# ooowedyn/InkLayer

Hardware: AMD Instinct MI355X
Metric: sketches/sec end-to-end (GroundingDINO+SAM) at 1024x1024 (higher is better)
Workload: dtype f16 (MFMA, f32 accumulate; f32 residual/norm/softmax; split-f16 = fp32-grade operands for patch-embed, neck, mask decoder)

## Files before the change

inklayer_amd/csrc/attention.hip:

```cpp
#include <stdlib.h>
#include "common.h"
#include "../../include/inklayer_hip.h"

int ink_win4_attn_launch(const InkAttn& p, int n_cus, hipStream_t s);
int ink_glob4_attn_launch(const InkAttn& p, hipStream_t s);

namespace {

typedef __attribute__((address_space(3))) s16x4* lds_s16x4_ptr;

__device__ __forceinline__ f16x4 tr_read(const char* p) {
  s16x4 v = __builtin_amdgcn_ds_read_tr16_b64_v4i16((lds_s16x4_ptr)(p));
  return __builtin_bit_cast(f16x4, v);
}

__device__ __forceinline__ f16x8 cvt8(const f32x16& s, int base) {
  f16x8 r;
#pragma unroll
  for (int j = 0; j < 8; ++j) r[j] = (f16)s[base + j];
  return r;
}

__device__ __forceinline__ float max3(float a, float b, float c) {
  float d;
  asm("v_max3_f32 %0, %1, %2, %3" : "=v"(d) : "v"(a), "v"(b), "v"(c));
  return d;
}

template <int HD, int MODE, int NW, bool ALLKV = false>
__global__ __launch_bounds__(NW * 64) void flash_attn_kernel(InkAttn p) {
  constexpr int NQKB = HD / 16;
  constexpr int NQK = NQKB + (MODE == 2 ? 2 : 0);
  constexpr int NB = (HD + 31) / 32;
  constexpr int DVP = NB * 32;
  constexpr bool LSUM_MFMA = DVP >= HD + 8;
  constexpr int CH = HD / 8;
  constexpr int KROW = ((NQK * 2) | 1) * 16;
  constexpr int VROW = DVP * 2;
  constexpr int NT = NW * 64;
  constexpr int KIT = (64 * CH + NT - 1) / NT;
  constexpr float NEG = -1e30f;
  constexpr int TILEB = 64 * KROW + 64 * VROW;
  constexpr int MAXT = ALLKV ? 4 : 2;
  extern __shared__ __attribute__((aligned(16))) char smem[];
  char* sK = smem;
  char* sV = smem + 64 * KROW;
  char* sR = smem + MAXT * TILEB;

  const int tid = threadIdx.x, lane = tid & 63, wave = tid >> 6;
  const int lq = lane & 31, hh = lane >> 5;
  const int nqb = (p.n_q + NW * 32 - 1) / (NW * 32);
  const int total = p.n_batch * p.n_heads * nqb;
  int blk = ALLKV ? (int)((int64_t)blockIdx.x * total / gridDim.x)
                  : (MODE == 1 ? xcd_remap((int)blockIdx.x, (int)gridDim.x) : (int)blockIdx.x);
  const int blk_end = ALLKV ? (int)((int64_t)(blockIdx.x + 1) * total / gridDim.x) : blk + 1;

  struct QState { bool ok; int64_t row; };
  constexpr int KALL = ALLKV ? (MAXT * 64 * CH + NT - 1) / NT : 1;
  int wrow_q = 0, wrow_k[KALL], wrow_b = -1;
  auto load_wrows = [&](int b_) {
    if (MODE == 2 && ALLKV && p.tok_rows && b_ != wrow_b) {
      const int qi = wave * 32 + lq;
      wrow_q = p.tok_rows[(int64_t)b_ * p.n_q + (qi < p.n_q ? qi : p.n_q - 1)];
#pragma unroll
      for (int it = 0; it < KALL; ++it) {
        const int key = (tid + it * NT) / CH;
        wrow_k[it] = key < p.n_k ? p.tok_rows[(int64_t)b_ * p.n_k + key] : -1;
      }
      wrow_b = b_;
    }
  };
  auto load_q = [&](int blk_, f16x8 (&dst)[NQK]) -> QState {
    const int bh_ = blk_ / nqb, qb_ = blk_ % nqb;
    const int b_ = bh_ / p.n_heads, h_ = bh_ % p.n_heads;
    const int qi = qb_ * NW * 32 + wave * 32 + lq;
    bool ok = qi < p.n_q;
    const int qc = ok ? qi : p.n_q - 1;
    const int64_t qrow0 = p.q_batch_rows ? (int64_t)p.q_batch_rows[b_] : (int64_t)b_ * p.n_q;
    int64_t row = qrow0 + qc;
    if constexpr (MODE == 2 && ALLKV) {
      if (p.tok_rows) {
        ok = ok && wrow_q >= 0;
        row = wrow_q >= 0 ? wrow_q : 0;
      }
    }
    const f16* Qrow = (const f16*)p.Q + row * p.ldq + h_ * HD;
#pragma unroll
    for (int s = 0; s < NQKB; ++s) dst[s] = *(const f16x8*)(Qrow + 16 * s + 8 * hh);
    if constexpr (MODE == 2) {
      const f16* R = (const f16*)p.rel_aug + ((int64_t)bh_ * p.n_q + qc) * 32;
      dst[NQKB] = *(const f16x8*)(R + 8 * hh);
      dst[NQKB + 1] = *(const f16x8*)(R + 16 + 8 * hh);
    }
    return QState{ok, row};
  };
  f16x8 ka[KALL], va[KALL];
  (void)ka; (void)va;
  auto load_kv_all = [&](int blk_) {
    const int bh_ = blk_ / nqb;
    const int b_ = bh_ / p.n_heads, h_ = bh_ % p.n_heads;
    const int64_t kvb_ = p.kv_batch_rows ? (int64_t)p.kv_batch_rows[b_] : (int64_t)b_ * p.n_k;
#pragma unroll
    for (int it = 0; it < KALL; ++it) {
      const int ci = tid + it * NT;
      const int key = ci / CH, cc = ci % CH;
      ka[it] = (f16x8){0, 0, 0, 0, 0, 0, 0, 0};
      va[it] = (f16x8){0, 0, 0, 0, 0, 0, 0, 0};
      if (ci < MAXT * 64 * CH && key < p.n_k) {
        int64_t r = kvb_ + key;
        if (MODE == 2 && p.tok_rows) r = wrow_k[it];
        if (r >= 0) {
          ka[it] = *(const f16x8*)((const f16*)p.K + r * p.ldk + h_ * HD + cc * 8);
          va[it] = *(const f16x8*)((const f16*)p.V + r * p.ldv + h_ * HD + cc * 8);
        } else {
          ka[it] = *(const f16x8*)((const f16*)p.pad_k + h_ * HD + cc * 8);
          va[it] = *(const f16x8*)((const f16*)p.pad_v + h_ * HD + cc * 8);
        }
      }
    }
  };
  load_wrows((blk / nqb) / p.n_heads);
  f16x8 qf[NQK];
  QState qs = load_q(blk, qf);
  if constexpr (ALLKV) load_kv_all(blk);
  if constexpr (DVP > HD) {
    constexpr int PCH = (DVP - HD) / 8;
    for (int i = tid; i < MAXT * 64 * PCH; i += NT) {
      const int row = (i / PCH) % 64, pc = i % PCH, tl = i / (64 * PCH);
      f16x8 z = {0, 0, 0, 0, 0, 0, 0, 0};
      if (LSUM_MFMA && pc == 0) { z[0] = (f16)1; z[4] = (f16)1; }
      *(f16x8*)(sV + tl * TILEB + row * VROW + (CH + pc) * 16) = z;
    }
  }
  int koff_g[KIT], voff_g[KIT], loff_k[KIT], loff_v[KIT];
#pragma unroll
  for (int it = 0; it < KIT; ++it) {
    const int ci = tid + it * NT;
    const int row = (ci / CH) & 63, cc = ci % CH;
    koff_g[it] = (row * (int)p.ldk + cc * 8) * 2;
    voff_g[it] = (row * (int)p.ldv + cc * 8) * 2;
    loff_k[it] = row * KROW + cc * 16;
    loff_v[it] = row * VROW + cc * 16;
  }
  if constexpr (MODE == 2 && ALLKV) {
    for (int i = tid; i < MAXT * 256; i += NT) {
      const int key = i >> 2, c4 = i & 3;
      const int kh = key / p.grid_w, kw = key - kh * p.grid_w + p.grid_w;
      f16x8 e;
#pragma unroll
      for (int j = 0; j < 8; ++j) {
        const int col = c4 * 8 + j;
        e[j] = (key < p.n_k && (col == kh || col == kw)) ? (f16)1 : (f16)0;
      }
      *(f16x8*)(sK + (key >> 6) * TILEB + (key & 63) * KROW + (CH + c4) * 16) = e;
    }
  }
  const float c = p.scale * 1.44269504088896340736f;
  const int ntiles = (p.n_k + 63) / 64;
  const bool half_tail = ALLKV && (p.n_k - (ntiles - 1) * 64) <= 32;
  const int koff0 = lq * KROW + hh * 16;
  const int koff1 = (32 + lq) * KROW + hh * 16;
  const int voff = (4 * hh + ((lane & 15) >> 2)) * VROW + (16 * ((lane >> 4) & 1) + 4 * (lane & 3)) * 2;
  constexpr int LI = HD / 32, LR = (((HD % 32) / 8) * 4);

  for (; blk < blk_end; ++blk) {
  const int bh = blk / nqb, qb = blk % nqb;
  const int b = bh / p.n_heads, h = bh % p.n_heads;
  const int q_idx = qb * NW * 32 + wave * 32 + lq;
  const int q_c = q_idx < p.n_q ? q_idx : p.n_q - 1;
  const bool q_ok = qs.ok;
  const int64_t q_row = qs.row;
  const int64_t kvb = p.kv_batch_rows ? (int64_t)p.kv_batch_rows[b] : (int64_t)b * p.n_k;
  const char* Kb = (const char*)((const f16*)p.K + kvb * p.ldk + h * HD);
  const char* Vb = (const char*)((const f16*)p.V + kvb * p.ldv + h * HD);
  float bias3[2][16];
  const float* RH = nullptr;
  if constexpr (MODE == 3) {
    const float* bp = p.dense_bias + ((int64_t)h * p.n_q + q_c) * 64;
    const float* mp = p.dense_mask ? p.dense_mask + ((int64_t)(b % p.n_mask) * p.n_q + q_c) * 64 : nullptr;
#pragma unroll
    for (int sub = 0; sub < 2; ++sub)
#pragma unroll
      for (int g = 0; g < 4; ++g) {
        f32x4 v = *(const f32x4*)(bp + sub * 32 + 8 * g + 4 * hh);
        if (mp) v += *(const f32x4*)(mp + sub * 32 + 8 * g + 4 * hh);
#pragma unroll
        for (int r = 0; r < 4; ++r) bias3[sub][4 * g + r] = v[r];
      }
  }
  f32x16 rw0, rw1;
  if constexpr (MODE == 1) {
    const float* RW = p.rel_w + ((int64_t)bh * p.n_q + q_c) * 64;
    RH = p.rel_h + ((int64_t)bh * p.n_q + q_c) * 64;
#pragma unroll
    for (int g = 0; g < 4; ++g) {
      const f32x4 a = *(const f32x4*)(RW + 8 * g + 4 * hh), c2 = *(const f32x4*)(RW + 32 + 8 * g + 4 * hh);
#pragma unroll
      for (int r = 0; r < 4; ++r) { rw0[4 * g + r] = a[r]; rw1[4 * g + r] = c2[r]; }
    }
  }

  f16x8 kreg[KIT], vreg[KIT];
  auto load_tile = [&](int t) {
    const char* kt = Kb + (int64_t)t * 64 * p.ldk * 2;
    const char* vt = Vb + (int64_t)t * 64 * p.ldv * 2;
    const bool full = (t + 1) * 64 <= p.n_k;
#pragma unroll
    for (int it = 0; it < KIT; ++it) {
      const int ci = tid + it * NT;
      const bool ok = ci < 64 * CH && (full || t * 64 + ci / CH < p.n_k);
      if (ok) {
        kreg[it] = *(const f16x8*)(kt + koff_g[it]);
        vreg[it] = *(const f16x8*)(vt + voff_g[it]);
      } else {
        kreg[it] = (f16x8){0, 0, 0, 0, 0, 0, 0, 0};
        vreg[it] = (f16x8){0, 0, 0, 0, 0, 0, 0, 0};
      }
    }
  };
  auto store_tile = [&](int t) {
#pragma unroll
    for (int it = 0; it < KIT; ++it) {
      if (tid + it * NT < 64 * CH) {
        *(f16x8*)(sK + (t & 1) * TILEB + loff_k[it]) = kreg[it];
        *(f16x8*)(sV + (t & 1) * TILEB + loff_v[it]) = vreg[it];
      }
    }
    if constexpr (MODE == 2 && !ALLKV) {
      for (int i = tid; i < 256; i += NT) {
        const int row = i >> 2, c4 = i & 3;
        const int key = t * 64 + row;
        const int kh = key / p.grid_w, kw = key - kh * p.grid_w + p.grid_w;
        f16x8 e;
#pragma unroll
        for (int j = 0; j < 8; ++j) {
          const int col = c4 * 8 + j;
          e[j] = (key < p.n_k && (col == kh || col == kw)) ? (f16)1 : (f16)0;
        }
        *(f16x8*)(sK + (t & 1) * TILEB + row * KROW + (CH + c4) * 16) = e;
      }
    }
  };

  f32x16 o[NB];
#pragma unroll
  for (int i = 0; i < NB; ++i)
#pragma unroll
    for (int r = 0; r < 16; ++r) o[i][r] = 0.f;
  float m_run = NEG, l_run = 0.f;

  float rh_next = 0.f;
  if constexpr (MODE == 1) rh_next = RH[0];
  if constexpr (ALLKV) {
    __syncthreads();
#pragma unroll
    for (int it = 0; it < KALL; ++it) {
      const int ci = tid + it * NT;
      const int key = ci / CH, cc = ci % CH;
      if (ci < MAXT * 64 * CH) {
        *(f16x8*)(sK + (key >> 6) * TILEB + (key & 63) * KROW + cc * 16) = ka[it];
        *(f16x8*)(sV + (key >> 6) * TILEB + (key & 63) * VROW + cc * 16) = va[it];
      }
    }
    __syncthreads();
    if (blk + 1 < blk_end) {
      load_wrows(((blk + 1) / nqb) / p.n_heads);
      load_kv_all(blk + 1);
    }
  } else {
    load_tile(0);
    store_tile(0);
    if (ntiles > 1) load_tile(1);
    __syncthreads();
  }
  const int nt_wave = (ALLKV && !__any(q_ok)) ? 0 : ntiles;
  for (int t = 0; t < nt_wave; ++t) {
    const char* tK = sK + (ALLKV ? t : (t & 1)) * TILEB;
    const char* tV = sV + (ALLKV ? t : (t & 1)) * TILEB;
    const float rh = rh_next;
    if constexpr (MODE == 1) {
      if (t + 1 < ntiles) rh_next = RH[t + 1];
    }

    f32x16 s0, s1;
    constexpr bool KPRE = !ALLKV;
    f16x8 kfa[KPRE ? NQK : 1], kfb[KPRE ? NQK : 1];
    if constexpr (KPRE) {
#pragma unroll
      for (int s = 0; s < NQK; ++s) {
        kfa[s] = *(const f16x8*)(tK + koff0 + s * 32);
        kfb[s] = *(const f16x8*)(tK + koff1 + s * 32);
      }
      __builtin_amdgcn_sched_barrier(0);
    }
    if constexpr (MODE == 1) {
      s0 = __builtin_amdgcn_mfma_f32_32x32x16_f16(kfa[0], qf[0], rw0, 0, 0, 0);
      s1 = __builtin_amdgcn_mfma_f32_32x32x16_f16(kfb[0], qf[0], rw1, 0, 0, 0);
    } else if constexpr (MODE == 3) {
#pragma unroll
      for (int r = 0; r < 16; ++r) {
        s0[r] = bias3[0][r];
        s1[r] = bias3[1][r];
      }
    } else {
#pragma unroll
      for (int r = 0; r < 16; ++r) s0[r] = s1[r] = 0.f;
    }
    const bool half = half_tail && t == ntiles - 1;
    if (half) {
#pragma unroll
      for (int s = 0; s < NQK; ++s) {
        const f16x8 k0 = *(const f16x8*)(tK + koff0 + s * 32);
        s0 = __builtin_amdgcn_mfma_f32_32x32x16_f16(k0, qf[s], s0, 0, 0, 0);
      }
    } else {
#pragma unroll
      for (int s = (MODE == 1 ? 1 : 0); s < NQK; ++s) {
        const f16x8 k0 = KPRE ? kfa[s] : *(const f16x8*)(tK + koff0 + s * 32);
        const f16x8 k1 = KPRE ? kfb[s] : *(const f16x8*)(tK + koff1 + s * 32);
        s0 = __builtin_amdgcn_mfma_f32_32x32x16_f16(k0, qf[s], s0, 0, 0, 0);
        s1 = __builtin_amdgcn_mfma_f32_32x32x16_f16(k1, qf[s], s1, 0, 0, 0);
      }
    }
    if ((t + 1) * 64 > p.n_k) {
#pragma unroll
      for (int r = 0; r < 16; ++r) {
        const int key = t * 64 + (r & 3) + 8 * (r >> 2) + 4 * hh;
        if (key >= p.n_k) s0[r] = NEG;
        if (key + 32 >= p.n_k) s1[r] = NEG;
      }
    }
    float mx = max3(s0[0], s0[1], s1[0]);
    mx = max3(mx, s1[1], s0[2]);
#pragma unroll
    for (int r = 3; r < 16; r += 2) mx = max3(mx, s0[r], s0[r + 1 < 16 ? r + 1 : r]);
#pragma unroll
    for (int r = 2; r < 16; r += 2) mx = max3(mx, s1[r], s1[r + 1]);
    mx = fmaxf(mx, __shfl_xor(mx, 32, 64));
    const float m_new = fmaxf(m_run, (mx + rh) * c);
    if (__any(m_new > m_run)) {
      const float alpha = __builtin_amdgcn_exp2f(m_run - m_new);
      l_run *= alpha;
#pragma unroll
      for (int i = 0; i < NB; ++i)
#pragma unroll
        for (int r = 0; r < 16; ++r) o[i][r] *= alpha;
      m_run = m_new;
    }
    const float koff = rh * c - m_run;
    f16x8 pf[4];
    auto pv = [&](int ks, int i) {
      const char* base = tV + voff + (16 * ks) * VROW + i * 64;
      const f16x4 a0 = tr_read(base);
      const f16x4 a1 = tr_read(base + 8 * VROW);
      const f16x8 vf = {a0[0], a0[1], a0[2], a0[3], a1[0], a1[1], a1[2], a1[3]};
      o[i] = __builtin_amdgcn_mfma_f32_32x32x16_f16(vf, pf[ks], o[i], 0, 0, 0);
    };
    if constexpr (LSUM_MFMA && !ALLKV) {
#pragma unroll
      for (int r = 0; r < 16; ++r) s0[r] = __builtin_amdgcn_exp2f(fmaf(s0[r], c, koff));
      pf[0] = cvt8(s0, 0);
      pf[1] = cvt8(s0, 8);
      if (half) {
#pragma unroll
        for (int ks = 0; ks < 2; ++ks)
#pragma unroll
          for (int i = 0; i < NB; ++i) pv(ks, i);
      } else {
        constexpr int NG = 2 * NB;
#pragma unroll
        for (int g = 0; g < NG; ++g) {
          pv(g / NB, g % NB);
#pragma unroll
          for (int r = (16 * g) / NG; r < (16 * (g + 1)) / NG; ++r) s1[r] = __builtin_amdgcn_exp2f(fmaf(s1[r], c, koff));
        }
        pf[2] = cvt8(s1, 0);
        pf[3] = cvt8(s1, 8);
#pragma unroll
        for (int ks = 2; ks < 4; ++ks)
#pragma unroll
          for (int i = 0; i < NB; ++i) pv(ks, i);
      }
    } else {
      float ps = 0.f;
#pragma unroll
      for (int r = 0; r < 16; ++r) {
        s0[r] = __builtin_amdgcn_exp2f(fmaf(s0[r], c, koff));
        s1[r] = __builtin_amdgcn_exp2f(fmaf(s1[r], c, koff));
        ps += s0[r] + s1[r];
      }
      if constexpr (!LSUM_MFMA) l_run += ps;
      pf[0] = cvt8(s0, 0);
      pf[1] = cvt8(s0, 8);
      pf[2] = cvt8(s1, 0);
      pf[3] = cvt8(s1, 8);
#pragma unroll
      for (int ks = 0; ks < 4; ++ks) {
        if (ks >= 2 && half) break;
#pragma unroll
        for (int i = 0; i < NB; ++i) pv(ks, i);
      }
    }
    if constexpr (!ALLKV) {
      if (t + 1 < ntiles) {
        store_tile(t + 1);
        if (t + 2 < ntiles) load_tile(t + 2);
      }
      __syncthreads();
    }
  }

  float ltot;
  if constexpr (LSUM_MFMA) {
    ltot = o[LI][LR];
  } else {
    ltot = l_run + __shfl_xor(l_run, 32, 64);
  }
  const float inv = 1.0f / ltot;
  if (q_ok) {
    const int64_t o_row = (MODE == 2 && ALLKV && p.tok_rows) ? q_row : (int64_t)b * p.n_q + q_idx;
    f16* Orow = (f16*)p.O + o_row * p.ldo + h * HD;
#pragma unroll
    for (int i = 0; i < NB; ++i)
#pragma unroll
      for (int g = 0; g < 4; ++g) {
        const int d0 = 32 * i + 8 * g + 4 * hh;
        if (d0 < HD) {
          const f16x4 v = {(f16)(o[i][4 * g] * inv), (f16)(o[i][4 * g + 1] * inv),
                           (f16)(o[i][4 * g + 2] * inv), (f16)(o[i][4 * g + 3] * inv)};
          *(f16x4*)(Orow + d0) = v;
        }
      }
  }
  if constexpr (ALLKV) {
    if (blk + 1 < blk_end) qs = load_q(blk + 1, qf);
  }
  }
}

template <int HD, int S, bool AUG, bool F16T = false>
__global__ __launch_bounds__(256) void relpos_mfma_kernel(const f16* __restrict__ Q, int64_t ldq,
                                                          const float* __restrict__ Rh,
                                                          const float* __restrict__ Rw, int n_heads,
                                                          float inv_scale, const int32_t* __restrict__ tok_rows,
                                                          float* __restrict__ out_h, float* __restrict__ out_w,
                                                          f16* __restrict__ out_aug) {
  constexpr int NQ = S * S;
  constexpr int RT = (2 * S - 1 + 31) / 32;
  constexpr int ROWS = 2 * RT * 32;
  constexpr int TROW = (HD / 8 + 1) * 16;
  constexpr int NQG = (NQ + 31) / 32;
  constexpr int GPB = AUG ? NQG : 8;
  constexpr int OROW = (AUG ? 64 : 256) + 16;
  __shared__ __attribute__((aligned(16))) char tab[ROWS * TROW + 4 * 32 * OROW];
  const int tid = threadIdx.x, lane = tid & 63, wave = tid >> 6;
  const int lq = lane & 31, hh = lane >> 5;
  char* ot = tab + ROWS * TROW + wave * 32 * OROW;
  const int nblk = (NQG + GPB - 1) / GPB;
  const int bh = blockIdx.x / nblk, gb = blockIdx.x % nblk;
  const int b = bh / n_heads, h = bh % n_heads;
  for (int i = tid; i < ROWS * (HD / 8); i += 256) {
    const int r = i / (HD / 8), c8 = i % (HD / 8);
    const int tr = r % (RT * 32);
    const float* src = (r < RT * 32 ? Rh : Rw) + (int64_t)tr * HD + c8 * 8;
    f16x8 v = {0, 0, 0, 0, 0, 0, 0, 0};
    if (tr < 2 * S - 1) {
      const f32x4 a = *(const f32x4*)src, c = *(const f32x4*)(src + 4);
      v = (f16x8){(f16)a[0], (f16)a[1], (f16)a[2], (f16)a[3], (f16)c[0], (f16)c[1], (f16)c[2], (f16)c[3]};
    }
    *(f16x8*)(tab + r * TROW + c8 * 16) = v;
  }
  __syncthreads();
  for (int g = gb * GPB + wave; g < min(NQG, (gb + 1) * GPB); g += 4) {
    const int q = g * 32 + lq;
    bool q_ok = q < NQ;
    const int qc = q_ok ? q : NQ - 1;
    int64_t qrow = (int64_t)b * NQ + qc;
    if (AUG && tok_rows) {
      const int r = tok_rows[qrow];
      q_ok = q_ok && r >= 0;
      qrow = r >= 0 ? r : 0;
    }
    const f16* qp = Q + qrow * ldq + h * HD;
    f16x8 qf[HD / 16];
#pragma unroll
    for (int s = 0; s < HD / 16; ++s) qf[s] = *(const f16x8*)(qp + 16 * s + 8 * hh);
    const int qh = qc / S, qw = qc % S;
    if (AUG && hh == 0) *(f16x4*)(ot + lq * OROW + 56) = (f16x4){0, 0, 0, 0};
#pragma unroll
    for (int tt = 0; tt < 2 * RT; ++tt) {
      f32x16 d;
#pragma unroll
      for (int r = 0; r < 16; ++r) d[r] = 0.f;
#pragma unroll
      for (int s = 0; s < HD / 16; ++s) {
        const f16x8 a = *(const f16x8*)(tab + (tt * 32 + lq) * TROW + (2 * s + hh) * 16);
        d = __builtin_amdgcn_mfma_f32_32x32x16_f16(a, qf[s], d, 0, 0, 0);
      }
      const bool is_w = tt >= RT;
      const int base = (is_w ? qw : qh) + S - 1 - (tt % RT) * 32;
#pragma unroll
      for (int r = 0; r < 16; ++r) {
        const int j = base - ((r & 3) + 8 * (r >> 2) + 4 * hh);
        if (j >= 0 && j < S) {
          const float v = d[r] * inv_scale;
          if (AUG) {
            *(f16*)(ot + lq * OROW + ((is_w ? S : 0) + j) * 2) = (f16)v;
          } else {
            *(float*)(ot + lq * OROW + j * 4) = v;
          }
        }
      }
      if (!AUG && (tt % RT) == RT - 1) {
        if (F16T) {
          f16* dst = (f16*)(is_w ? out_w : out_h) + ((int64_t)bh * NQ + q) * S + hh * 32;
          if (q_ok) {
#pragma unroll
            for (int i = 0; i < 4; ++i) {
              const f32x4 a = *(const f32x4*)(ot + lq * OROW + hh * 128 + i * 32), c = *(const f32x4*)(ot + lq * OROW + hh * 128 + i * 32 + 16);
              *(f16x8*)(dst + 8 * i) = (f16x8){(f16)a[0], (f16)a[1], (f16)a[2], (f16)a[3], (f16)c[0], (f16)c[1], (f16)c[2], (f16)c[3]};
            }
          }
        } else {
          float* dst = (is_w ? out_w : out_h) + ((int64_t)bh * NQ + q) * S + hh * 32;
          if (q_ok) {
#pragma unroll
            for (int i = 0; i < 8; ++i) *(f32x4*)(dst + 4 * i) = *(const f32x4*)(ot + lq * OROW + hh * 128 + i * 16);
          }
        }
      }
    }
    if (AUG && q_ok) {
      f16* dst = out_aug + ((int64_t)bh * NQ + q) * 32 + hh * 16;
      *(f16x8*)dst = *(const f16x8*)(ot + lq * OROW + hh * 32);
      *(f16x8*)(dst + 8) = *(const f16x8*)(ot + lq * OROW + hh * 32 + 16);
    }
  }
}

}

extern "C" int ink_flash_attn(const InkAttn* pp, void* stream) {
  INK_CHECK_ARG(pp != nullptr);
  const InkAttn& p = *pp;
  INK_CHECK_ARG(p.Q && p.K && p.V && p.O);
  INK_CHECK_ARG(p.n_batch > 0 && p.n_heads > 0 && p.n_q > 0 && p.n_k > 0);
  INK_CHECK_ARG(p.ldq % 8 == 0 && p.ldk % 8 == 0 && p.ldv % 8 == 0 && p.ldo % 4 == 0);
  INK_CHECK_ARG((((uintptr_t)p.Q | (uintptr_t)p.K | (uintptr_t)p.V) & 15) == 0);
  INK_CHECK_ARG(((uintptr_t)p.O & 7) == 0);
  INK_CHECK_ARG(!p.tok_rows || p.bias_mode == 2);
  static const int n_cus = [] {
    int dev = 0, n = 0;
    if (hipGetDevice(&dev) != hipSuccess || hipDeviceGetAttribute(&n, hipDeviceAttributeMultiprocessorCount, dev) != hipSuccess || n <= 0) n = 256;
    return n;
  }();
  constexpr bool persist = true;
  hipStream_t s = (hipStream_t)stream;
  const int bhn = p.n_batch * p.n_heads;
#define INK_FA_X(HD, MODE, NW, ALL)                                                                      \
  {                                                                                                        \
    constexpr int nqk_ = HD / 16 + (MODE == 2 ? 2 : 0);                                                    \
    constexpr int lds_ = (ALL ? 4 : 2) * (64 * (((nqk_ * 2) | 1) * 16) + 64 * (((HD + 31) / 32) * 64)) +   \
                         0;                                                                            \
    static bool attr_ = ((void)hipFuncSetAttribute((const void*)flash_attn_kernel<HD, MODE, NW, ALL>,      \
                                                   hipFuncAttributeMaxDynamicSharedMemorySize, lds_), true); \
    (void)attr_;                                                                                           \
    const int nqb = (p.n_q + NW * 32 - 1) / (NW * 32);                                                     \
    const int grid_ = (ALL && persist) ? (bhn * nqb < n_cus ? bhn * nqb : n_cus) : bhn * nqb;                \
    hipLaunchKernelGGL((flash_attn_kernel<HD, MODE, NW, ALL>), dim3(grid_), dim3(NW * 64), lds_, s, p);      \
  }
#define INK_FA(HD, MODE, NW) INK_FA_X(HD, MODE, NW, false)
  if (p.head_dim == 80 && p.bias_mode == 1) {
    INK_CHECK_ARG(p.rel_h && p.rel_w && p.grid_w == 64 && p.n_k % 64 == 0);
    if (p.n_q % 256 == 0 && p.n_k % 128 == 0 && p.n_k >= 256 && p.n_k <= 4096) return ink_glob4_attn_launch(p, s);
    INK_CHECK_ARG(!p.rel_f16);
    INK_FA(80, 1, 8);
  } else if (p.head_dim == 80 && p.bias_mode == 2) {
    INK_CHECK_ARG(p.rel_aug && p.grid_w > 0 && p.grid_w <= 16 && p.n_k <= p.grid_w * p.grid_w && p.n_k <= 256);
    INK_CHECK_ARG(!p.tok_rows || (p.n_q == p.n_k && p.pad_k && p.pad_v &&
                                  (((uintptr_t)p.pad_k | (uintptr_t)p.pad_v) & 15) == 0));
    if (p.n_k >= 193 && p.n_k <= 208 && p.n_q <= 256 &&
        (p.tok_rows || (int64_t)p.n_batch * p.n_q * p.ldo * 2 < 0x80000000LL))
      return ink_win4_attn_launch(p, n_cus, s);
    INK_FA_X(80, 2, 7, true);
  } else if (p.head_dim == 80 && p.bias_mode == 0) {
    INK_FA(80, 0, 4);
  } else if (p.head_dim == 64 && p.bias_mode == 0) {
    INK_FA(64, 0, 4);
  } else if (p.head_dim == 32 && p.bias_mode == 0) {
    if (p.n_q <= 32) { INK_FA(32, 0, 1) } else { INK_FA(32, 0, 4) }
  } else if (p.head_dim == 32 && p.bias_mode == 3) {
    INK_CHECK_ARG(p.dense_bias && p.n_k <= 64 && p.n_q <= 64 && (!p.dense_mask || p.n_mask > 0));
    INK_FA(32, 3, 2);
  } else if (p.head_dim == 16 && p.bias_mode == 0) {
    if (p.n_q <= 32) { INK_FA(16, 0, 1) } else { INK_FA(16, 0, 4) }
  } else {
    return INK_ERR_ARG;
  }
#undef INK_FA
#undef INK_FA_X
  return ink_launch_status();
}

extern "C" int ink_relpos_bias64_f16(const void* Q, int64_t ldq, const float* rel_pos_h, const float* rel_pos_w,
                                     int32_t n_batch, int32_t n_heads, int32_t head_dim, float scale, void* out_h_f16,
                                     void* out_w_f16, void* stream) {
  INK_CHECK_ARG(Q && rel_pos_h && rel_pos_w && head_dim == 80 && ldq % 8 == 0 && out_h_f16 && out_w_f16);
  INK_CHECK_ARG(n_batch > 0 && n_heads > 0 && scale > 0.f && ((((uintptr_t)out_h_f16 | (uintptr_t)out_w_f16) & 15) == 0));
  hipLaunchKernelGGL((relpos_mfma_kernel<80, 64, false, true>), dim3(n_batch * n_heads * 16), dim3(256), 0, (hipStream_t)stream,
                     (const f16*)Q, ldq, rel_pos_h, rel_pos_w, n_heads, 1.0f / scale, (const int32_t*)nullptr,
                     (float*)out_h_f16, (float*)out_w_f16, (f16*)nullptr);
  return ink_launch_status();
}

extern "C" int ink_relpos_bias(const void* Q, int64_t ldq, const float* rel_pos_h,
                               const float* rel_pos_w, int32_t S, int32_t n_batch,
                               int32_t n_heads, int32_t head_dim, float scale, const int32_t* tok_rows,
                               float* out_h, float* out_w, void* out_aug_f16, void* stream) {
  INK_CHECK_ARG(Q && rel_pos_h && rel_pos_w && head_dim == 80 && ldq % 8 == 0);
  INK_CHECK_ARG(n_batch > 0 && n_heads > 0 && S > 0 && scale > 0.f);
  if (out_aug_f16) {
    INK_CHECK_ARG(S <= 16);
  } else {
    INK_CHECK_ARG(S == 64 && out_h && out_w && !tok_rows);
  }
  const f16* q = (const f16*)Q;
  hipStream_t st = (hipStream_t)stream;
  const int nbh = n_batch * n_heads;
  if (out_aug_f16) {
    INK_CHECK_ARG(S == 14);
    hipLaunchKernelGGL((relpos_mfma_kernel<80, 14, true>), dim3(nbh), dim3(256), 0, st, q, ldq, rel_pos_h,
                       rel_pos_w, n_heads, 1.0f / scale, tok_rows, out_h, out_w, (f16*)out_aug_f16);
  } else {
    hipLaunchKernelGGL((relpos_mfma_kernel<80, 64, false>), dim3(nbh * 16), dim3(256), 0, st, q, ldq, rel_pos_h,
                       rel_pos_w, n_heads, 1.0f / scale, (const int32_t*)nullptr, out_h, out_w, (f16*)nullptr);
  }
  return ink_launch_status();
}
```

inklayer_amd/csrc/common.h:

```cpp
#pragma once
#include <hip/hip_runtime.h>
#include <stdint.h>

typedef _Float16 f16;
typedef _Float16 f16x2 __attribute__((ext_vector_type(2)));
typedef _Float16 f16x4 __attribute__((ext_vector_type(4)));
typedef _Float16 f16x8 __attribute__((ext_vector_type(8)));
typedef float f32x2 __attribute__((ext_vector_type(2)));
typedef float f32x4 __attribute__((ext_vector_type(4)));
typedef float f32x16 __attribute__((ext_vector_type(16)));
typedef short s16x4 __attribute__((ext_vector_type(4)));

#define INK_OK 0
#define INK_ERR_ARG 1
#define INK_ERR_LAUNCH 2

#define INK_CHECK_ARG(cond)            \
  do {                                 \
    if (!(cond)) return INK_ERR_ARG;   \
  } while (0)

static inline int ink_launch_status() {
  hipError_t e = hipGetLastError();
  return e == hipSuccess ? INK_OK : INK_ERR_LAUNCH;
}

__device__ __forceinline__ float wave_sum(float v) {
#pragma unroll
  for (int o = 32; o > 0; o >>= 1) v += __shfl_xor(v, o, 64);
  return v;
}
__device__ __forceinline__ float wave_max(float v) {
#pragma unroll
  for (int o = 32; o > 0; o >>= 1) v = fmaxf(v, __shfl_xor(v, o, 64));
  return v;
}

__device__ __forceinline__ float gelu_erf(float x) {
  const float u = fabsf(x) * 0.84932180028801904272f;
  const float t = __builtin_amdgcn_rcpf(fmaf(0.27273748087922250f, u, 1.0f));
  float pl = fmaf(1.061405429f, t, -1.453152027f);
  pl = fmaf(pl, t, 1.421413741f);
  pl = fmaf(pl, t, -0.284496736f);
  pl = fmaf(pl, t, 0.254829592f);
  const float e = pl * t * __builtin_amdgcn_exp2f(-(u * u));
  return fmaf(-0.5f * fabsf(x), e, fmaxf(x, 0.0f));
}

__device__ __forceinline__ int xcd_remap(int bid, int nwg) {
  const int q = nwg >> 3, r = nwg & 7, x = bid & 7;
  return (x < r ? x * (q + 1) : r * (q + 1) + (x - r) * q) + (bid >> 3);
}
```

inklayer_amd/csrc/norm.hip:

```cpp
#include "common.h"
#include "../../include/inklayer_hip.h"

namespace {

__device__ __forceinline__ void split_store(f16* o, int C, const f32x4& y) {
  f16x4 hi, lo, hs;
#pragma unroll
  for (int e = 0; e < 4; ++e) {
    hi[e] = (f16)y[e];
    lo[e] = (f16)((y[e] - (float)hi[e]) * 64.0f);
    hs[e] = (f16)((float)hi[e] * 0.015625f);
  }
  *(f16x4*)o = hi;
  *(f16x4*)(o + C) = lo;
  *(f16x4*)(o + 2 * C) = hs;
}

template <int NV>
__global__ __launch_bounds__(256) void layernorm_rows_kernel(
    const float* __restrict__ x, int64_t ldx, const float* __restrict__ gamma,
    const float* __restrict__ beta, float eps, const int32_t* __restrict__ gather, int rows_out,
    int C, f16* __restrict__ out_h, float* __restrict__ out_f, int64_t ldo, int act, int split,
    const float* __restrict__ add, int64_t ld_add, const int32_t* __restrict__ add_batch_rows, int rows_per_batch) {
  const int lane = threadIdx.x & 63;
  const int row = blockIdx.x * 4 + (threadIdx.x >> 6);
  if (row >= rows_out) return;
  const int nv = C >> 2;
  const int64_t ldf = split ? ldo / 3 : ldo;
  const int src = gather ? gather[row] : row;
  if (src < 0) {
    for (int v = lane; v < nv; v += 64) {
      if (out_h && split) split_store(out_h + row * ldo + v * 4, C, (f32x4){0.f, 0.f, 0.f, 0.f});
      else if (out_h) *(f16x4*)(out_h + row * ldo + v * 4) = (f16x4){0, 0, 0, 0};
      if (out_f) *(f32x4*)(out_f + row * ldf + v * 4) = (f32x4){0.f, 0.f, 0.f, 0.f};
    }
    return;
  }
  const float* xr = x + (int64_t)src * ldx;
  const float* ar = nullptr;
  if (add) {
    const int b = row / rows_per_batch, i = row - b * rows_per_batch;
    ar = add + ((int64_t)(add_batch_rows ? add_batch_rows[b] : b * rows_per_batch) + i) * ld_add;
  }
  f32x4 r[NV];
  float s = 0.f;
#pragma unroll
  for (int j = 0; j < NV; ++j) {
    const int v = lane + 64 * j;
    r[j] = v < nv ? *(const f32x4*)(xr + v * 4) : (f32x4){0.f, 0.f, 0.f, 0.f};
    if (ar && v < nv) r[j] += *(const f32x4*)(ar + v * 4);
    s += (r[j][0] + r[j][1]) + (r[j][2] + r[j][3]);
  }
  const float mean = wave_sum(s) / (float)C;
  float q = 0.f;
#pragma unroll
  for (int j = 0; j < NV; ++j) {
    const int v = lane + 64 * j;
    if (v < nv) {
      const f32x4 d = r[j] - mean;
      q += (d[0] * d[0] + d[1] * d[1]) + (d[2] * d[2] + d[3] * d[3]);
    }
  }
  const float rstd = 1.0f / sqrtf(wave_sum(q) / (float)C + eps);
#pragma unroll
  for (int j = 0; j < NV; ++j) {
    const int v = lane + 64 * j;
    if (v < nv) {
      f32x4 y = (r[j] - mean) * rstd;
      if (gamma) y *= *(const f32x4*)(gamma + v * 4);
      if (beta) y += *(const f32x4*)(beta + v * 4);
      if (act == INK_ACT_GELU) {
#pragma unroll
        for (int e = 0; e < 4; ++e) y[e] = gelu_erf(y[e]);
      }
      if (out_h && split) split_store(out_h + row * ldo + v * 4, C, y);
      else if (out_h) *(f16x4*)(out_h + row * ldo + v * 4) = (f16x4){(f16)y[0], (f16)y[1], (f16)y[2], (f16)y[3]};
      if (out_f) *(f32x4*)(out_f + row * ldf + v * 4) = y;
    }
  }
}

__global__ __launch_bounds__(256) void add_split_f16_kernel(const float* __restrict__ a,
                                                            const float* __restrict__ b,
                                                            f16* __restrict__ o, int64_t n4, int64_t nb4,
                                                            int C) {
  const int c4n = C >> 2;
  for (int64_t i = blockIdx.x * 256 + threadIdx.x; i < n4; i += (int64_t)gridDim.x * 256) {
    f32x4 v = *(const f32x4*)(a + i * 4);
    if (b) v += *(const f32x4*)(b + (i % nb4) * 4);
    const int64_t row = i / c4n;
    const int c = (int)(i - row * c4n) * 4;
    split_store(o + row * 3 * C + c, C, v);
  }
}

__global__ __launch_bounds__(256) void add_cvt_f16_kernel(const float* __restrict__ a,
                                                          const float* __restrict__ b,
                                                          f16* __restrict__ o,
                                                          float* __restrict__ of, int64_t n4,
                                                          int64_t nb4) {
  for (int64_t i = blockIdx.x * 256 + threadIdx.x; i < n4; i += (int64_t)gridDim.x * 256) {
    f32x4 v = *(const f32x4*)(a + i * 4);
    if (b) v += *(const f32x4*)(b + (i % nb4) * 4);
    if (o) *(f16x4*)(o + i * 4) = (f16x4){(f16)v[0], (f16)v[1], (f16)v[2], (f16)v[3]};
    if (of) *(f32x4*)(of + i * 4) = v;
  }
}

}

extern "C" int ink_layernorm_rows(const float* x, int64_t ldx, const float* gamma,
                                  const float* beta, float eps, const int32_t* gather,
                                  int32_t rows_out, int32_t C, void* out_f16, float* out_f32,
                                  int64_t ldo, int32_t act, int32_t split, const float* add, int64_t ld_add,
                                  const int32_t* add_batch_rows, int32_t rows_per_batch, void* stream) {
  INK_CHECK_ARG(x && (out_f16 || out_f32));
  INK_CHECK_ARG(!add || (!gather && rows_per_batch > 0 && ld_add >= C && ld_add % 4 == 0));
  INK_CHECK_ARG(split == 0 || (split == 1 && out_f16 && ldo >= 3 * (int64_t)C && (!out_f32 || ldo % 12 == 0)));
  INK_CHECK_ARG(act == INK_ACT_NONE || act == INK_ACT_GELU);
  INK_CHECK_ARG(rows_out > 0 && C > 0 && C % 4 == 0 && C <= 2048);
  INK_CHECK_ARG(ldx % 4 == 0 && ldo % 4 == 0 && ldx >= C && ldo >= C);
  const dim3 grid((rows_out + 3) / 4), block(256);
  hipStream_t s = (hipStream_t)stream;
  const int nv = (C / 4 + 63) / 64;
#define INK_LN(NV)                                                                          \
  hipLaunchKernelGGL(layernorm_rows_kernel<NV>, grid, block, 0, s, x, ldx, gamma, beta, eps, \
                     gather, rows_out, C, (f16*)out_f16, out_f32, ldo, act, split, add, ld_add, add_batch_rows, \
                     rows_per_batch)
  switch (nv) {
    case 1: INK_LN(1); break;
    case 2: INK_LN(2); break;
    case 3: INK_LN(3); break;
    case 4: INK_LN(4); break;
    case 5: INK_LN(5); break;
    default: INK_LN(8); break;
  }
#undef INK_LN
  return ink_launch_status();
}

extern "C" int ink_add_cvt_f16(const float* a, const float* b, int64_t n_b, void* out_f16,
                               int64_t n, void* stream) {
  INK_CHECK_ARG(a && out_f16 && n > 0 && n % 4 == 0);
  INK_CHECK_ARG(!b || (n_b > 0 && n_b % 4 == 0 && n % n_b == 0));
  const int64_t n4 = n / 4;
  const int blocks = (int)((n4 + 255) / 256 < 2048 ? (n4 + 255) / 256 : 2048);
  hipLaunchKernelGGL(add_cvt_f16_kernel, dim3(blocks), dim3(256), 0, (hipStream_t)stream, a, b,
                     (f16*)out_f16, (float*)nullptr, n4, b ? n_b / 4 : 1);
  return ink_launch_status();
}

extern "C" int ink_add_split_f16(const float* a, const float* b, int64_t n_b, void* out_f16, int64_t n,
                                 int32_t C, void* stream) {
  INK_CHECK_ARG(a && out_f16 && n > 0 && C > 0 && C % 4 == 0 && n % C == 0);
  INK_CHECK_ARG(!b || (n_b > 0 && n_b % 4 == 0 && n % n_b == 0));
  const int64_t n4 = n / 4;
  const int blocks = (int)((n4 + 255) / 256 < 4096 ? (n4 + 255) / 256 : 4096);
  hipLaunchKernelGGL(add_split_f16_kernel, dim3(blocks), dim3(256), 0, (hipStream_t)stream, a, b,
                     (f16*)out_f16, n4, b ? n_b / 4 : 1, C);
  return ink_launch_status();
}

extern "C" int ink_add_f32(const float* a, const float* b, int64_t n_b, float* out, int64_t n,
                           void* stream) {
  INK_CHECK_ARG(a && out && n > 0 && n % 4 == 0);
  INK_CHECK_ARG(!b || (n_b > 0 && n_b % 4 == 0 && n % n_b == 0));
  const int64_t n4 = n / 4;
  const int blocks = (int)((n4 + 255) / 256 < 2048 ? (n4 + 255) / 256 : 2048);
  hipLaunchKernelGGL(add_cvt_f16_kernel, dim3(blocks), dim3(256), 0, (hipStream_t)stream, a, b,
                     (f16*)nullptr, out, n4, b ? n_b / 4 : 1);
  return ink_launch_status();
}
```

Before: 117.3.

## Use persistent grid-stride kernels for relpos bias and C=1280 layernorm

Replaces the one-block-per-tile relpos MFMA launch with a persistent kernel: each wave walks a contiguous range of query-group tasks, builds the f16 rel-pos table in LDS once per block, and prefetches the next task's Q rows while computing the current one. Adds a persistent, software-prefetching layernorm path for C=1280 f16 output that keeps gamma/beta in registers and loads the next row early. Both aim to cut repeated table setup, launch/tail overhead and exposed load latency, in exchange for more register pressure and possible load imbalance. CU-count lookup is also factored into a shared helper.

```diff
diff --git a/inklayer_amd/csrc/attention.hip b/inklayer_amd/csrc/attention.hip
--- a/inklayer_amd/csrc/attention.hip
+++ b/inklayer_amd/csrc/attention.hip
@@ -435,6 +435,120 @@
   if constexpr (ALLKV) {
     if (blk + 1 < blk_end) qs = load_q(blk + 1, qf);
   }
+  }
+}
+
+template <int HD, int S, bool AUG, bool F16T = false>
+__global__ __launch_bounds__(256, 2) void relpos_walk_kernel(const f16* __restrict__ Q, int64_t ldq,
+                                                          const float* __restrict__ Rh,
+                                                          const float* __restrict__ Rw, int n_heads,
+                                                          float inv_scale, const int32_t* __restrict__ tok_rows,
+                                                          float* __restrict__ out_h, float* __restrict__ out_w,
+                                                          f16* __restrict__ out_aug, int n_tasks) {
+  constexpr int NQ = S * S;
+  constexpr int RT = (2 * S - 1 + 31) / 32;
+  constexpr int ROWS = 2 * RT * 32;
+  constexpr int TROW = (HD / 8 + 1) * 16;
+  constexpr int TAB = ROWS * TROW;
+  constexpr int NQG = (NQ + 31) / 32;
+  constexpr int NS = HD / 16;
+  constexpr int OROW = (AUG ? 64 : 256) + 16;
+  __shared__ __attribute__((aligned(16))) char tab[TAB + 4 * 32 * OROW];
+  const int tid = threadIdx.x, lane = tid & 63, wave = tid >> 6;
+  const int lq = lane & 31, hh = lane >> 5;
+  char* ot = tab + TAB + wave * 32 * OROW;
+  for (int i = tid; i < ROWS * (HD / 8); i += 256) {
+    const int r = i / (HD / 8), c8 = i % (HD / 8);
+    const int tr = r % (RT * 32);
+    const float* src = (r < RT * 32 ? Rh : Rw) + (int64_t)tr * HD + c8 * 8;
+    f16x8 v = {0, 0, 0, 0, 0, 0, 0, 0};
+    if (tr < 2 * S - 1) {
+      const f32x4 a = *(const f32x4*)src, c = *(const f32x4*)(src + 4);
+      v = (f16x8){(f16)a[0], (f16)a[1], (f16)a[2], (f16)a[3], (f16)c[0], (f16)c[1], (f16)c[2], (f16)c[3]};
+    }
+    *(f16x8*)(tab + r * TROW + c8 * 16) = v;
+  }
+  __syncthreads();
+  const int64_t gw = blockIdx.x * 4 + wave, nw = (int64_t)gridDim.x * 4;
+  int t = __builtin_amdgcn_readfirstlane((int)(gw * n_tasks / nw));
+  const int t_end = __builtin_amdgcn_readfirstlane((int)((gw + 1) * n_tasks / nw));
+  if (t >= t_end) return;
+  const auto src_row = [&](int task) -> int {
+    const int bh = task / NQG, g = task - bh * NQG;
+    const int q = g * 32 + lq;
+    const int row = (bh / n_heads) * NQ + (q < NQ ? q : NQ - 1);
+    return (AUG && tok_rows) ? tok_rows[row] : row;
+  };
+  const auto load_q = [&](int task, int row, f16x8* qf) {
+    const f16* qp = Q + (int64_t)(row >= 0 ? row : 0) * ldq + ((task / NQG) % n_heads) * HD;
+#pragma unroll
+    for (int s = 0; s < NS; ++s) qf[s] = *(const f16x8*)(qp + 16 * s + 8 * hh);
+  };
+  int r_cur = src_row(t);
+  int r_nxt = src_row(t + 1 < t_end ? t + 1 : t);
+  f16x8 qf[NS], qn[NS];
+  load_q(t, r_cur, qn);
+  for (; t < t_end; ++t) {
+#pragma unroll
+    for (int s = 0; s < NS; ++s) qf[s] = qn[s];
+    load_q(t + 1 < t_end ? t + 1 : t, r_nxt, qn);
+    const int r_nn = src_row(t + 2 < t_end ? t + 2 : t_end - 1);
+    const int bh = t / NQG, g = t - bh * NQG;
+    const int q = g * 32 + lq;
+    const bool q_ok = q < NQ && r_cur >= 0;
+    const int qc = q < NQ ? q : NQ - 1;
+    const int qh = qc / S, qw = qc % S;
+    if (AUG && hh == 0) *(f16x4*)(ot + lq * OROW + 56) = (f16x4){0, 0, 0, 0};
+#pragma unroll
+    for (int tt = 0; tt < 2 * RT; ++tt) {
+      f32x16 d;
+#pragma unroll
+      for (int r = 0; r < 16; ++r) d[r] = 0.f;
+#pragma unroll
+      for (int s = 0; s < NS; ++s) {
+        const f16x8 a = *(const f16x8*)(tab + (tt * 32 + lq) * TROW + (2 * s + hh) * 16);
+        d = __builtin_amdgcn_mfma_f32_32x32x16_f16(a, qf[s], d, 0, 0, 0);
+      }
+      const bool is_w = tt >= RT;
+      const int base = (is_w ? qw : qh) + S - 1 - (tt % RT) * 32;
+#pragma unroll
+      for (int r = 0; r < 16; ++r) {
+        const int j = base - ((r & 3) + 8 * (r >> 2) + 4 * hh);
+        if (j >= 0 && j < S) {
+          const float v = d[r] * inv_scale;
+          if (AUG) {
+            *(f16*)(ot + lq * OROW + ((is_w ? S : 0) + j) * 2) = (f16)v;
+          } else {
+            *(float*)(ot + lq * OROW + j * 4) = v;
+          }
+        }
+      }
+      if (!AUG && (tt % RT) == RT - 1) {
+        if (F16T) {
+          f16* dst = (f16*)(is_w ? out_w : out_h) + ((int64_t)bh * NQ + q) * S + hh * 32;
+          if (q_ok) {
+#pragma unroll
+            for (int i = 0; i < 4; ++i) {
+              const f32x4 a = *(const f32x4*)(ot + lq * OROW + hh * 128 + i * 32), c = *(const f32x4*)(ot + lq * OROW + hh * 128 + i * 32 + 16);
+              *(f16x8*)(dst + 8 * i) = (f16x8){(f16)a[0], (f16)a[1], (f16)a[2], (f16)a[3], (f16)c[0], (f16)c[1], (f16)c[2], (f16)c[3]};
+            }
+          }
+        } else {
+          float* dst = (is_w ? out_w : out_h) + ((int64_t)bh * NQ + q) * S + hh * 32;
+          if (q_ok) {
+#pragma unroll
+            for (int i = 0; i < 8; ++i) *(f32x4*)(dst + 4 * i) = *(const f32x4*)(ot + lq * OROW + hh * 128 + i * 16);
+          }
+        }
+      }
+    }
+    if (AUG && q_ok) {
+      f16* dst = out_aug + ((int64_t)bh * NQ + q) * 32 + hh * 16;
+      *(f16x8*)dst = *(const f16x8*)(ot + lq * OROW + hh * 32);
+      *(f16x8*)(dst + 8) = *(const f16x8*)(ot + lq * OROW + hh * 32 + 16);
+    }
+    r_cur = r_nxt;
+    r_nxt = r_nn;
   }
 }
 
@@ -538,6 +652,11 @@
   }
 }
 
+static inline int relpos_grid(int64_t n_tasks, int wgs_per_cu) {
+  const int64_t full = (int64_t)ink_cu_count() * wgs_per_cu, need = (n_tasks + 3) / 4;
+  return (int)(need < full ? need : full);
+}
+
 }
 
 extern "C" int ink_flash_attn(const InkAttn* pp, void* stream) {
@@ -549,11 +668,7 @@
   INK_CHECK_ARG((((uintptr_t)p.Q | (uintptr_t)p.K | (uintptr_t)p.V) & 15) == 0);
   INK_CHECK_ARG(((uintptr_t)p.O & 7) == 0);
   INK_CHECK_ARG(!p.tok_rows || p.bias_mode == 2);
-  static const int n_cus = [] {
-    int dev = 0, n = 0;
-    if (hipGetDevice(&dev) != hipSuccess || hipDeviceGetAttribute(&n, hipDeviceAttributeMultiprocessorCount, dev) != hipSuccess || n <= 0) n = 256;
-    return n;
-  }();
+  const int n_cus = ink_cu_count();
   constexpr bool persist = true;
   hipStream_t s = (hipStream_t)stream;
   const int bhn = p.n_batch * p.n_heads;
@@ -607,9 +722,11 @@
                                      void* out_w_f16, void* stream) {
   INK_CHECK_ARG(Q && rel_pos_h && rel_pos_w && head_dim == 80 && ldq % 8 == 0 && out_h_f16 && out_w_f16);
   INK_CHECK_ARG(n_batch > 0 && n_heads > 0 && scale > 0.f && ((((uintptr_t)out_h_f16 | (uintptr_t)out_w_f16) & 15) == 0));
-  hipLaunchKernelGGL((relpos_mfma_kernel<80, 64, false, true>), dim3(n_batch * n_heads * 16), dim3(256), 0, (hipStream_t)stream,
+  INK_CHECK_ARG((int64_t)n_batch * n_heads * 128 < 0x7fffffffLL);
+  const int n_tasks = n_batch * n_heads * 128;
+  hipLaunchKernelGGL((relpos_walk_kernel<80, 64, false, true>), dim3(relpos_grid(n_tasks, 2)), dim3(256), 0, (hipStream_t)stream,
                      (const f16*)Q, ldq, rel_pos_h, rel_pos_w, n_heads, 1.0f / scale, (const int32_t*)nullptr,
-                     (float*)out_h_f16, (float*)out_w_f16, (f16*)nullptr);
+                     (float*)out_h_f16, (float*)out_w_f16, (f16*)nullptr, n_tasks);
   return ink_launch_status();
 }
 
@@ -626,14 +743,16 @@
   }
   const f16* q = (const f16*)Q;
   hipStream_t st = (hipStream_t)stream;
-  const int nbh = n_batch * n_heads;
+  const int64_t nbh = (int64_t)n_batch * n_heads;
+  INK_CHECK_ARG(nbh * 128 < 0x7fffffffLL);
   if (out_aug_f16) {
     INK_CHECK_ARG(S == 14);
-    hipLaunchKernelGGL((relpos_mfma_kernel<80, 14, true>), dim3(nbh), dim3(256), 0, st, q, ldq, rel_pos_h,
+    hipLaunchKernelGGL((relpos_mfma_kernel<80, 14, true>), dim3((int)nbh), dim3(256), 0, st, q, ldq, rel_pos_h,
                        rel_pos_w, n_heads, 1.0f / scale, tok_rows, out_h, out_w, (f16*)out_aug_f16);
   } else {
-    hipLaunchKernelGGL((relpos_mfma_kernel<80, 64, false>), dim3(nbh * 16), dim3(256), 0, st, q, ldq, rel_pos_h,
-                       rel_pos_w, n_heads, 1.0f / scale, (const int32_t*)nullptr, out_h, out_w, (f16*)nullptr);
+    const int n_tasks = (int)nbh * 128;
+    hipLaunchKernelGGL((relpos_walk_kernel<80, 64, false>), dim3(relpos_grid(n_tasks, 2)), dim3(256), 0, st, q, ldq, rel_pos_h,
+                       rel_pos_w, n_heads, 1.0f / scale, (const int32_t*)nullptr, out_h, out_w, (f16*)nullptr, n_tasks);
   }
   return ink_launch_status();
 }
diff --git a/inklayer_amd/csrc/common.h b/inklayer_amd/csrc/common.h
--- a/inklayer_amd/csrc/common.h
+++ b/inklayer_amd/csrc/common.h
@@ -23,6 +23,15 @@
 static inline int ink_launch_status() {
   hipError_t e = hipGetLastError();
   return e == hipSuccess ? INK_OK : INK_ERR_LAUNCH;
+}
+
+static inline int ink_cu_count() {
+  static const int n_cus = [] {
+    int dev = 0, n = 0;
+    if (hipGetDevice(&dev) != hipSuccess || hipDeviceGetAttribute(&n, hipDeviceAttributeMultiprocessorCount, dev) != hipSuccess || n <= 0) n = 256;
+    return n;
+  }();
+  return n_cus;
 }
 
 __device__ __forceinline__ float wave_sum(float v) {
diff --git a/inklayer_amd/csrc/norm.hip b/inklayer_amd/csrc/norm.hip
--- a/inklayer_amd/csrc/norm.hip
+++ b/inklayer_amd/csrc/norm.hip
@@ -80,6 +80,52 @@
   }
 }
 
+template <int NV>
+__global__ __launch_bounds__(256) void layernorm_stream_kernel(const float* __restrict__ x, int64_t ldx,
+                                                               const float* __restrict__ gamma,
+                                                               const float* __restrict__ beta, float eps, int rows,
+                                                               f16* __restrict__ out_h, int64_t ldo) {
+  constexpr int C = NV * 256;
+  const int lane = threadIdx.x & 63;
+  const int n_waves = gridDim.x * 4;
+  int row = blockIdx.x * 4 + (threadIdx.x >> 6);
+  if (row >= rows) return;
+  f32x4 g[NV], bt[NV], nx[NV];
+#pragma unroll
+  for (int j = 0; j < NV; ++j) {
+    nx[j] = *(const f32x4*)(x + (int64_t)row * ldx + (lane + 64 * j) * 4);
+    g[j] = *(const f32x4*)(gamma + (lane + 64 * j) * 4);
+    bt[j] = *(const f32x4*)(beta + (lane + 64 * j) * 4);
+  }
+  for (; row < rows; row += n_waves) {
+    f32x4 r[NV];
+#pragma unroll
+    for (int j = 0; j < NV; ++j) r[j] = nx[j];
+    const int nrow = row + n_waves < rows ? row + n_waves : row;
+#pragma unroll
+    for (int j = 0; j < NV; ++j) nx[j] = *(const f32x4*)(x + (int64_t)nrow * ldx + (lane + 64 * j) * 4);
+    float s = 0.f;
+#pragma unroll
+    for (int j = 0; j < NV; ++j) s += (r[j][0] + r[j][1]) + (r[j][2] + r[j][3]);
+    const float mean = wave_sum(s) / (float)C;
+    float q = 0.f;
+#pragma unroll
+    for (int j = 0; j < NV; ++j) {
+      const f32x4 d = r[j] - mean;
+      q += (d[0] * d[0] + d[1] * d[1]) + (d[2] * d[2] + d[3] * d[3]);
+    }
+    const float rstd = 1.0f / sqrtf(wave_sum(q) / (float)C + eps);
+    f16* o = out_h + (int64_t)row * ldo;
+#pragma unroll
+    for (int j = 0; j < NV; ++j) {
+      f32x4 y = (r[j] - mean) * rstd;
+      y *= g[j];
+      y += bt[j];
+      *(f16x4*)(o + (lane + 64 * j) * 4) = (f16x4){(f16)y[0], (f16)y[1], (f16)y[2], (f16)y[3]};
+    }
+  }
+}
+
 __global__ __launch_bounds__(256) void add_split_f16_kernel(const float* __restrict__ a,
                                                             const float* __restrict__ b,
                                                             f16* __restrict__ o, int64_t n4, int64_t nb4,
@@ -122,6 +168,12 @@
   INK_CHECK_ARG(ldx % 4 == 0 && ldo % 4 == 0 && ldx >= C && ldo >= C);
   const dim3 grid((rows_out + 3) / 4), block(256);
   hipStream_t s = (hipStream_t)stream;
+  if (C == 1280 && gamma && beta && !gather && !add && !split && act == INK_ACT_NONE && out_f16 && !out_f32) {
+    const int blocks = grid.x < (unsigned)ink_cu_count() * 4 ? (int)grid.x : ink_cu_count() * 4;
+    hipLaunchKernelGGL(layernorm_stream_kernel<5>, dim3(blocks), block, 0, s, x, ldx, gamma, beta, eps, rows_out,
+                       (f16*)out_f16, ldo);
+    return ink_launch_status();
+  }
   const int nv = (C / 4 + 63) / 64;
 #define INK_LN(NV)                                                                          \
   hipLaunchKernelGGL(layernorm_rows_kernel<NV>, grid, block, 0, s, x, ldx, gamma, beta, eps, \
```

After: 118.0, median of 6. No clear change (+0.6%).
